# xenji/kafka-topic-analyzer

Measured on NVIDIA H100. Metric: messages/sec scanned (fused metric scan), higher is better.
Workload: dtype u64

## Files before the change

### kafka_topic_analyzer_b200/csrc/kta_api.cu

```cuda
#include <cuda_runtime.h>

#include <algorithm>
#include <chrono>
#include <climits>
#include <cmath>
#include <cstdarg>
#include <cstdio>
#include <cstdlib>
#include <cstring>
#include <new>
#include <vector>

#include "kta_host.cuh"
#include "kta_kernels.cuh"
#include "kta_logscan.cuh"
#include "kta_partitioner.cuh"
#include "kta_synth.h"
#include "kta_timeline.cuh"

using namespace kta;

extern "C" const char *kta_last_error(void) { return g_err; }
extern "C" int kta_abi_version(void) { return KTA_ABI_VERSION; }
extern "C" int kta_device_count(void) {
// ... 50 lines not shown
    int32_t buckets = 0;
    int64_t origin = 0, width = 1;
    bool smem = false;
    int blocks_per_sm = 0;
    DevBuf<unsigned long long> d_bins;
    std::vector<uint64_t> h_bins;
    size_t words() const { return d_bins.cap > 0 ? (size_t)d_bins.cap : 0; }
};

struct Partitioner {
    int32_t ncounts = 0;
    int32_t counts[KTA_PARTITIONER_MAX_COUNTS] = {};
    bool smem = false;
    int32_t max_grid = 0;
    DevBuf<unsigned long long> d_counts;
    std::vector<uint64_t> h_counts;
    size_t words() const { return d_counts.cap > 0 ? (size_t)d_counts.cap : 0; }
};

struct kta_handle {
    kta_config cfg{};
    int device = 0;
    int sm_count = 0;
    cudaStream_t stream = nullptr;
    bool own_stream = true;
    bool need_hash = false;
    DevBuf<unsigned long long> d_sums;
    DevBuf<long long> d_minmax;
    DevBuf<uint32_t> d_hll;
    DevBuf<uint32_t> d_hll_floor;
    AliveKeys alive;
    uint32_t *d_hash_out = nullptr;
    DevBuf<uint64_t> d_tb_scratch;
    LogScan log;
    Timeline tl;
    Partitioner pt;
    DevBuf<uint32_t> d_crc32_tables;
    size_t nsums = 0, nhll = 0;
    Chunk chunks[NCHUNK];
    bool ring_dev_ready = false, ring_host_ready = false;
    int64_t ring_records = 0, ring_key_bytes = 0;
    int cur = 0;
    struct PushCursor {
        int32_t *part = nullptr, *klen = nullptr, *vlen = nullptr;
        int64_t *ts = nullptr;
        uint8_t *keys = nullptr;
        uint64_t *tile_base = nullptr;
        int64_t n = 0, cap = 0;
        int64_t kb = 0, kcap = 0;
        bool hash = false;
    } pc;
    uint64_t next_seq = 0;
    bool finalized = false;
    std::vector<uint64_t> h_sums;
    long long h_minmax[4] = {0, 0, 0, 0};
    std::vector<uint32_t> h_hll;
    uint64_t h_alive = 0;
    int shard_world = 1, shard_rank = 0;
    int columns = 0;
    bool smem_counters = true;
    size_t smem_optin = 0;
    uint64_t launches = 0, records = 0;
    bool timing = false;
    std::vector<std::pair<cudaEvent_t, cudaEvent_t>> ev_pool;
    size_t ev_used = 0;
    double scan_ms = 0;
    uint64_t scan_launches_timed = 0;
};

static int set_device(const kta_handle *h) {
    CU(cudaSetDevice(h->device));
    return KTA_OK;
}

static bool keys_travel(const kta_handle *h) { return h->need_hash || h->d_hash_out || h->pt.ncounts; }

static size_t scan_smem_bytes(bool hash, bool smem, int P, int threads, int keybuf, int stages, bool hdr) {
    return (smem ? smem_counter_bytes(P) : CTA_SCRATCH) + (size_t)(threads / 32) * warp_smem_bytes(hash, keybuf, stages, hdr);
}

static void scan_shape(const kta_handle *h, bool hash, bool hdr_ok, int64_t n, int64_t key_bytes, int &threads, int &keybuf,
                       int &stages, bool &hdr, size_t &smem) {
    const int P = h->columns;
    keybuf = KEYBUF_MIN;
    stages = 0;
    hdr = false;
    if (!hash) {
        threads = MAX_THREADS;
        smem = scan_smem_bytes(false, h->smem_counters, P, threads, keybuf, stages, hdr);
        return;
    }
    if (n > 0) {
        const int64_t per_tile = (key_bytes * TILE + n - 1) / n;
        int64_t want = per_tile + per_tile / 8 + 64 + KEYBUF_SLACK;
        want = (want + 127) / 128 * 128;
        keybuf = (int)std::min<int64_t>(std::max<int64_t>(want, KEYBUF_MIN), KEYBUF_MAX);
        keybuf = (keybuf + 15) / 16 * 16;
    }
    auto fits = [&](bool with_hdr, int st, int max_warps, int min_warps) {
        hdr = with_hdr;
        stages = st;
        for (threads = std::min(max_warps * 32, HASH_MAX_THREADS); threads >= min_warps * 32; threads -= 32) {
            smem = scan_smem_bytes(true, h->smem_counters, P, threads, keybuf, stages, hdr);
            if (smem <= h->smem_optin) return true;
        }
        return false;
    };
    if (hdr_ok && (fits(true, SCAN_STAGES, 12, 10) || fits(true, 2, 12, 10))) return;
    if (fits(false, 2, 16, 8)) return;
// ... 251 lines not shown
    if (!h) return KTA_OK;
    cudaSetDevice(h->device);
    if (h->stream) cudaStreamSynchronize(h->stream);
    for (auto &c : h->chunks)
        if (c.free_ev) cudaEventDestroy(c.free_ev);
    for (auto &e : h->ev_pool) { cudaEventDestroy(e.first); cudaEventDestroy(e.second); }
    cudaStream_t own = h->own_stream ? h->stream : nullptr;
    delete h;
    if (own) cudaStreamDestroy(own);
    cudaGetLastError();
    return KTA_OK;
}

static int create_impl(const kta_config *cfg, kta_handle *h) {
    h->cfg = *cfg;
    if (cfg->num_partitions < 1 || cfg->num_partitions > (1 << 20))
        return fail(KTA_ERR_INVALID, "num_partitions %d out of range [1, 2^20]", cfg->num_partitions);
    if (cfg->hll_precision != 0 && (cfg->hll_precision < 4 || cfg->hll_precision > 18))
        return fail(KTA_ERR_INVALID, "hll_precision %d not 0 or 4..18", cfg->hll_precision);
    if (cfg->isolation_level != KTA_READ_UNCOMMITTED && cfg->isolation_level != KTA_READ_COMMITTED)
        return fail(KTA_ERR_INVALID, "isolation_level %d is neither KTA_READ_UNCOMMITTED (0) nor KTA_READ_COMMITTED (1)", cfg->isolation_level);
    int ndev = 0;
    CU(cudaGetDeviceCount(&ndev));
    if (ndev < 1) return fail(KTA_ERR_CUDA, "no CUDA device (this library has no CPU fallback)");
    if (cfg->device >= 0) h->device = cfg->device;
    else CU(cudaGetDevice(&h->device));
    if (h->device >= ndev) return fail(KTA_ERR_INVALID, "device %d >= device count %d", h->device, ndev);
    CU(cudaSetDevice(h->device));
    cudaDeviceProp prop;
    CU(cudaGetDeviceProperties(&prop, h->device));
    if (prop.major != 9 || prop.minor != 0) return fail(KTA_ERR_CUDA, "device %s is sm_%d%d; this library is built for sm_90a only",
                                     prop.name, prop.major, prop.minor);
    h->sm_count = prop.multiProcessorCount;
    CU(cudaStreamCreateWithFlags(&h->stream, cudaStreamNonBlocking));
    h->need_hash = cfg->count_alive_keys == 1 || cfg->hll_precision != 0;
    h->pc.hash = keys_travel(h);
    if (cfg->now_s == INT64_MIN) {
        const auto now = std::chrono::system_clock::now().time_since_epoch();
        const int64_t ns = std::chrono::duration_cast<std::chrono::nanoseconds>(now).count();
        h->cfg.now_s = ns / 1000000000ll;
        h->cfg.now_ns = (int32_t)(ns % 1000000000ll);
    }
    h->ring_records = cfg->ring_records > 0 ? cfg->ring_records : DEFAULT_RING_RECORDS;
    h->ring_records = (h->ring_records + TILE - 1) / TILE * TILE;
    h->ring_key_bytes = cfg->ring_key_bytes > 0 ? cfg->ring_key_bytes : h->ring_records * 24;

    const int P = cfg->num_partitions;
    h->nsums = sums_words(P);
    h->nhll = cfg->hll_precision ? ((size_t)1 << cfg->hll_precision) : 0;
    int rc;
    if ((rc = h->d_sums.alloc((int64_t)h->nsums)) || (rc = h->d_minmax.alloc(4)) || (rc = h->d_hll_floor.alloc(HLL_SLICES + 2)))
        return rc;
    if (h->nhll && (rc = h->d_hll.alloc((int64_t)h->nhll))) return rc;
    if (cfg->count_alive_keys == 1 && (rc = alive_create(h))) return rc;
    h->smem_optin = prop.sharedMemPerBlockOptin;
    if (cfg->shard_world > 1) {
        if (cfg->shard_rank < 0 || cfg->shard_rank >= cfg->shard_world || cfg->shard_world > P)
            return fail(KTA_ERR_INVALID, "shard_rank %d / shard_world %d invalid for %d partitions", cfg->shard_rank, cfg->shard_world, P);
        const uint64_t G = (uint64_t)cfg->shard_world, e = (((uint64_t)1 << 32) + G - 1) / G * G - ((uint64_t)1 << 32);
        if ((uint64_t)(P - 1) * e >= (uint64_t)1 << 32)
            return fail(KTA_ERR_INVALID, "shard_world %d with %d partitions: the scan's partition division is exact only when "
                        "(P - 1) * (ceil(2^32 / G) * G - 2^32) < 2^32 (every P <= 65536 and every G <= 4096 qualify)",
                        cfg->shard_world, P);
        h->shard_world = cfg->shard_world;
        h->shard_rank = cfg->shard_rank;
    }
    h->columns = (P - h->shard_rank + h->shard_world - 1) / h->shard_world;
    h->smem_counters = smem_counter_bytes(h->columns) + 8 * warp_smem_bytes(true, KEYBUF_MIN, 2, false) <= h->smem_optin;
    for (const auto &by_mode : SCAN_KERNELS[h->smem_counters])
        for (const auto &by_capture : by_mode)
            for (const ScanFn f : by_capture)
                if (f) CU(cudaFuncSetAttribute(f, cudaFuncAttributeMaxDynamicSharedMemorySize, (int)h->smem_optin));
    if ((rc = log_scan_create(h->log, cfg->isolation_level == KTA_READ_COMMITTED, h->smem_optin))) return rc;
    if ((rc = state_reset_device(h))) return rc;
    CU(cudaStreamSynchronize(h->stream));
    return KTA_OK;
}

extern "C" int kta_create(const kta_config *cfg, kta_handle **out) {
    if (!cfg || !out) return fail(KTA_ERR_INVALID, "null argument");
    if (cfg->struct_size != (int32_t)sizeof(kta_config))
        return fail(KTA_ERR_INVALID, "kta_config.struct_size %d != %zu (ABI version %d)", cfg->struct_size, sizeof(kta_config), KTA_ABI_VERSION);
    kta_handle *h = new (std::nothrow) kta_handle();
    if (!h) return fail(KTA_ERR_NOMEM, "out of host memory");
    const int rc = create_impl(cfg, h);
    if (rc) {
        char keep[sizeof(g_err)];
        memcpy(keep, g_err, sizeof(keep));
        kta_destroy(h);
        memcpy(g_err, keep, sizeof(keep));
        *out = nullptr;
        return rc;
    }
    *out = h;
    return KTA_OK;
}

extern "C" void *kta_stream(kta_handle *h) { return h ? (void *)h->stream : nullptr; }

extern "C" int kta_set_stream(kta_handle *h, void *stream) {
    if (!h) return fail(KTA_ERR_INVALID, "null handle");
    int rc;
    if ((rc = set_device(h))) return rc;
    CU(cudaStreamSynchronize(h->stream));
    if (h->own_stream) CU(cudaStreamDestroy(h->stream));
    h->stream = (cudaStream_t)stream;
// ... 617 lines not shown
    if ((rc = collect_timing(h))) return rc;
    h->next_seq = std::max<uint64_t>(h->next_seq, seq_base + (uint64_t)b->n);
    return KTA_OK;
}

extern "C" int kta_sync(kta_handle *h) {
    if (!h) return fail(KTA_ERR_INVALID, "null handle");
    int rc;
    if ((rc = set_device(h))) return rc;
    if ((rc = ring_flush(h))) return rc;
    CU(cudaStreamSynchronize(h->stream));
    if ((rc = alive_settle(h))) return rc;
    return collect_timing(h);
}

extern "C" int kta_reset(kta_handle *h) {
    if (!h) return fail(KTA_ERR_INVALID, "null handle");
    int rc;
    if ((rc = set_device(h))) return rc;
    h->pc.n = 0;
    h->pc.kb = 0;
    h->next_seq = 0;
    h->finalized = false;
    h->launches = 0;
    h->records = 0;
    h->log.txn.ranges.clear();
    for (uint64_t &v : h->log.txn.totals) v = 0;
    for (uint64_t &v : h->log.crc.totals) v = 0;
    h->log.crc.kept.clear();
    OffsetState &o = h->log.offsets;
    std::fill(o.win.begin(), o.win.end(), make_longlong2(-1, -1));
    o.set = 0;
    o.dirty = !o.win.empty();
    for (uint64_t &v : o.totals) v = 0;
    if (h->tl.buckets) CU(cudaMemsetAsync(h->tl.d_bins, 0, h->tl.words() * 8, h->stream));
    if (h->pt.ncounts) CU(cudaMemsetAsync(h->pt.d_counts, 0, h->pt.words() * 8, h->stream));
    return state_reset_device(h);
}

extern "C" int kta_finalize(kta_handle *h) {
    if (!h) return fail(KTA_ERR_INVALID, "null handle");
    int rc;
    if ((rc = set_device(h))) return rc;
    if ((rc = ring_flush(h))) return rc;
    cudaStream_t s = h->stream;
    if ((rc = alive_settle(h))) return rc;
    if (h->alive.d_table && h->nhll) {
        CU(cudaMemsetAsync(h->d_hll, 0, h->nhll * 4, s));
        alive_hll_kernel<<<h->sm_count * 8, THREADS, 0, s>>>(h->alive.d_table, (size_t)h->alive.pairs * 2, h->d_hll,
                                                             h->cfg.hll_precision);
        CU(cudaGetLastError());
        h->launches++;
    }
    h->h_sums.resize(h->nsums);
    h->h_hll.resize(h->nhll);
    CU(cudaMemcpyAsync(h->h_sums.data(), h->d_sums, h->nsums * 8, cudaMemcpyDeviceToHost, s));
    CU(cudaMemcpyAsync(h->h_minmax, h->d_minmax, 32, cudaMemcpyDeviceToHost, s));
    if (h->nhll) CU(cudaMemcpyAsync(h->h_hll.data(), h->d_hll, h->nhll * 4, cudaMemcpyDeviceToHost, s));
    if (h->tl.buckets) {
        h->tl.h_bins.resize(h->tl.words());
        CU(cudaMemcpyAsync(h->tl.h_bins.data(), h->tl.d_bins, h->tl.words() * 8, cudaMemcpyDeviceToHost, s));
    }
    if (h->pt.ncounts) {
        h->pt.h_counts.resize(h->pt.words());
        CU(cudaMemcpyAsync(h->pt.h_counts.data(), h->pt.d_counts, h->pt.words() * 8, cudaMemcpyDeviceToHost, s));
    }
    CU(cudaStreamSynchronize(s));
    if ((rc = collect_timing(h))) return rc;
    h->h_alive = h->alive.now;
    h->finalized = true;
    if (h->alive.window_errors)
        return fail(KTA_ERR_INVALID, "%llu record(s) carried a sequence number outside the alive-key table's window "
                    "[origin, origin + 2^31 - 2): with an explicit seq column the span between kta_reset calls is limited",
                    (unsigned long long)h->alive.window_errors);
    const uint64_t bad = h->h_sums[h->nsums - 1];
    if (bad)
        return fail(KTA_ERR_PARTITION, "%llu record(s) had a partition outside [0, %d) and were left out of every metric",
                    (unsigned long long)bad, h->cfg.num_partitions);
    return KTA_OK;
}

static int check_read(const kta_handle *h, int32_t p, bool per_partition) {
    if (!h) return fail(KTA_ERR_INVALID, "null handle");
    if (!h->finalized) return fail(KTA_ERR_NOT_FINALIZED, "call kta_finalize first");
    if (per_partition && (p < 0 || p >= h->cfg.num_partitions)) return -1;
    return KTA_OK;
}

static uint64_t raw_counter(const kta_handle *h, int which, int32_t p) {
    const int P = h->cfg.num_partitions;
    const uint64_t *s = h->h_sums.data();
    uint64_t knn = 0, alive = 0;
    for (int b = 0; b < NB; b++) {
        knn += s[(size_t)p * NB + b];
        alive += s[(size_t)(P + p) * NB + b];
    }
    const uint64_t knull = s[(size_t)P * (2 * NB + 2) + p];
    const uint64_t total = knn + knull;
    switch (which) {
        case KTA_TOTAL: return total;
        case KTA_TOMBSTONES: return total - alive;
        case KTA_ALIVE: return alive;
        case KTA_KEY_NULL: return knull;
        case KTA_KEY_NON_NULL: return knn;
        case KTA_KEY_SIZE_SUM: return s[(size_t)P * (2 * NB) + p];
        case KTA_VALUE_SIZE_SUM: return s[(size_t)P * (2 * NB + 1) + p];
    }
    return 0;
}

extern "C" int kta_counter(const kta_handle *h, int which, int32_t partition, uint64_t *out) {
    if (!out || which < 0 || which > KTA_VALUE_SIZE_SUM) return fail(KTA_ERR_INVALID, "bad argument");
    const int rc = check_read(h, partition, true);
    if (rc > 0) return rc;
    *out = rc < 0 ? 0 : raw_counter(h, which, partition);
    return KTA_OK;
}

extern "C" int kta_avg(const kta_handle *h, int which, int32_t partition, uint64_t *out) {
    if (!out || which < 0 || which > KTA_MESSAGE_SIZE_AVG) return fail(KTA_ERR_INVALID, "bad argument");
    const int rc = check_read(h, partition, true);
    if (rc > 0) return rc;
    if (rc < 0) { *out = 0; return KTA_OK; }
    const uint64_t ks = raw_counter(h, KTA_KEY_SIZE_SUM, partition), vs = raw_counter(h, KTA_VALUE_SIZE_SUM, partition);
    const uint64_t alive = raw_counter(h, KTA_ALIVE, partition);
    const uint64_t sum = which == KTA_KEY_SIZE_AVG ? ks : which == KTA_VALUE_SIZE_AVG ? vs : ks + vs;
    if (sum > 0) {
        if (alive == 0)
            return fail(KTA_ERR_DIV_BY_ZERO, "partition %d: sum %llu > 0 with alive == 0 (the reference panics here)",
                        partition, (unsigned long long)sum);
        *out = sum / alive;
    } else {
        *out = 0;
    }
    return KTA_OK;
}

extern "C" int kta_dirty_ratio(const kta_handle *h, int32_t partition, float *out) {
    if (!out) return fail(KTA_ERR_INVALID, "bad argument");
    const int rc = check_read(h, partition, true);
    if (rc > 0) return rc;
    *out = 0.0f;
    if (rc < 0) return KTA_OK;
    const uint64_t total = raw_counter(h, KTA_TOTAL, partition), tomb = raw_counter(h, KTA_TOMBSTONES, partition);
    if (total > 0 && tomb > 0) {
        const volatile float t = (float)tomb;
        const volatile float d = (float)total / 100.0f;
        *out = t / d;
    }
    return KTA_OK;
}

extern "C" int kta_global(const kta_handle *h, int which, uint64_t *out) {
    if (!out) return fail(KTA_ERR_INVALID, "bad argument");
    const int rc = check_read(h, 0, false);
    if (rc) return rc;
    const int P = h->cfg.num_partitions;
    const unsigned long long *mm = reinterpret_cast<const unsigned long long *>(h->h_minmax);
    switch (which) {
        case KTA_SMALLEST_MESSAGE: *out = mm[2] == ~0ull ? 0 : mm[2]; return KTA_OK;
        case KTA_LARGEST_MESSAGE: *out = mm[3]; return KTA_OK;
        case KTA_OVERALL_SIZE: {
            uint64_t s = 0;
            for (int p = 0; p < P; p++) s += raw_counter(h, KTA_KEY_SIZE_SUM, p) + raw_counter(h, KTA_VALUE_SIZE_SUM, p);
            *out = s;
            return KTA_OK;
        }
        case KTA_OVERALL_COUNT: {
            uint64_t s = 0;
            for (int p = 0; p < P; p++) s += raw_counter(h, KTA_TOTAL, p);
            *out = s;
            return KTA_OK;
        }
    }
    return fail(KTA_ERR_INVALID, "bad global id %d", which);
}

extern "C" int kta_timestamps(const kta_handle *h, int64_t *earliest_s, int32_t *earliest_ns, int64_t *latest_s) {
    const int rc = check_read(h, 0, false);
    if (rc) return rc;
    int64_t es = h->cfg.now_s, ls = 0;
    int32_t ens = h->cfg.now_ns;
    if (h->h_minmax[0] != INT64_MAX) {
        const int64_t raw_mn = h->h_minmax[0] == -1 ? 0 : h->h_minmax[0];
        const int64_t raw_mx = h->h_minmax[1] == -1 ? 0 : h->h_minmax[1];
        const int64_t mn = raw_mn / 1000, mx = raw_mx / 1000;
        if (es > mn || (es == mn && ens > 0)) { es = mn; ens = 0; }
        if (ls < mx) ls = mx;
    }
    if (earliest_s) *earliest_s = es;
    if (earliest_ns) *earliest_ns = ens;
    if (latest_s) *latest_s = ls;
    return KTA_OK;
}

extern "C" int kta_alive_keys(const kta_handle *h, uint64_t *out) {
    if (!out) return fail(KTA_ERR_INVALID, "bad argument");
    const int rc = check_read(h, 0, false);
    if (rc) return rc;
    if (h->cfg.count_alive_keys != 1) return fail(KTA_ERR_NOT_ENABLED, "count_alive_keys was not enabled");
    *out = h->h_alive;
    return KTA_OK;
}

extern "C" int kta_bad_partition_records(const kta_handle *h, uint64_t *out) {
    if (!out) return fail(KTA_ERR_INVALID, "bad argument");
    const int rc = check_read(h, 0, false);
    if (rc) return rc;
    *out = h->h_sums[h->nsums - 1];
    return KTA_OK;
}
// ... 121 lines not shown
    if (!h || cap < 0 || (cap && !out)) return fail(KTA_ERR_INVALID, "bad argument");
    if (!h->pt.ncounts) return fail(KTA_ERR_NOT_ENABLED, "the partitioner check is off (kta_set_partitioner_check)");
    const int rc = check_read(h, partition, true);
    if (rc > 0) return rc;
    const int64_t nv = 2 * (int64_t)h->pt.ncounts + 1, n = std::min<int64_t>(cap, nv);
    for (int64_t b = 0; b < n; b++)
        out[b] = rc < 0 ? 0 : h->pt.h_counts[(size_t)b * (size_t)h->cfg.num_partitions + (size_t)partition];
    return KTA_OK;
}

extern "C" int kta_partitioner_shape(const kta_handle *h, int64_t n, int64_t key_bytes, int32_t *grid, int32_t *stage,
                                     int32_t *smem_counters) {
    if (!h || n < 0 || !grid || !stage || !smem_counters) return fail(KTA_ERR_INVALID, "bad argument");
    if (!h->pt.ncounts) return fail(KTA_ERR_NOT_ENABLED, "the partitioner check is off (kta_set_partitioner_check)");
    int rc;
    if ((rc = set_device(h))) return rc;
    int g = 0, st = 0;
    size_t sm = 0;
    if ((rc = partitioner_shape(h, n, key_bytes, g, st, sm))) return rc;
    *grid = g;
    *stage = st;
    *smem_counters = h->pt.smem ? 1 : 0;
    return KTA_OK;
}

extern "C" int kta_partitioner_limit_grid(kta_handle *h, int32_t max_ctas) {
    if (!h || max_ctas < 0) return fail(KTA_ERR_INVALID, "bad argument");
    if (!h->pt.ncounts) return fail(KTA_ERR_NOT_ENABLED, "the partitioner check is off (kta_set_partitioner_check)");
    h->pt.max_grid = max_ctas;
    return KTA_OK;
}

static double hll_sigma(double x) {
    if (x == 1.0) return INFINITY;
    double y = 1.0, z = x, zo;
    do { x *= x; zo = z; z += x * y; y += y; } while (zo != z);
    return z;
}
static double hll_tau(double x) {
    if (x == 0.0 || x == 1.0) return 0.0;
    double y = 1.0, z = 1.0 - x, zo;
    do { x = std::sqrt(x); zo = z; y *= 0.5; z -= (1.0 - x) * (1.0 - x) * y; } while (zo != z);
    return z / 3.0;
}

extern "C" int kta_alive_keys_hll(const kta_handle *h, double *out) {
    if (!out) return fail(KTA_ERR_INVALID, "bad argument");
    const int rc = check_read(h, 0, false);
    if (rc) return rc;
    if (!h->nhll) return fail(KTA_ERR_NOT_ENABLED, "hll_precision was 0");
    const int p = h->cfg.hll_precision, q = 32 - p;
    const double m = (double)h->nhll;
    std::vector<double> C((size_t)q + 2, 0.0);
    for (uint32_t r : h->h_hll) C[std::min<uint32_t>(r, (uint32_t)q + 1)] += 1.0;
    double z = m * hll_tau(1.0 - C[(size_t)q + 1] / m);
    for (int k = q; k >= 1; k--) z = 0.5 * (z + C[(size_t)k]);
    z += m * hll_sigma(C[0] / m);
    *out = 0.72134752044448170368 * m * m / z;
    return KTA_OK;
}

extern "C" int kta_hll_registers(const kta_handle *h, uint8_t *out, size_t cap) {
    if (!out) return fail(KTA_ERR_INVALID, "bad argument");
    const int rc = check_read(h, 0, false);
    if (rc) return rc;
    if (!h->nhll) return fail(KTA_ERR_NOT_ENABLED, "hll_precision was 0");
    if (cap < h->nhll) return fail(KTA_ERR_INVALID, "buffer too small: %zu < %zu", cap, h->nhll);
    for (size_t i = 0; i < h->nhll; i++) out[i] = (uint8_t)h->h_hll[i];
    return KTA_OK;
}

extern "C" int kta_fnv32_host(kta_handle *h, int64_t n, const int32_t *key_len, const uint8_t *key_bytes,
                              int64_t key_bytes_len, uint32_t *out) {
    if (!h || n < 0 || (n && (!key_len || !out))) return fail(KTA_ERR_INVALID, "bad argument");
    if (n == 0) return KTA_OK;
    int rc;
    if ((rc = set_device(h))) return rc;
    std::vector<uint64_t> off((size_t)n);
    uint64_t acc = 0;
    for (int64_t i = 0; i < n; i++) {
        off[(size_t)i] = acc;
        acc += key_len[i] > 0 ? (uint64_t)key_len[i] : 0;
    }
    if ((int64_t)acc > key_bytes_len) return fail(KTA_ERR_INVALID, "key_bytes_len %lld < sum of key_len %llu",
                                                  (long long)key_bytes_len, (unsigned long long)acc);
    DevBuf<int32_t> d_len;
    DevBuf<uint64_t> d_off;
    DevBuf<uint8_t> d_keys;
    DevBuf<uint32_t> d_out;
    cudaStream_t s = h->stream;
    if ((rc = d_len.alloc(n)) || (rc = d_off.alloc(n)) || (rc = d_keys.alloc((int64_t)acc + 16)) || (rc = d_out.alloc(n))) return rc;
    CU(cudaMemcpyAsync(d_len, key_len, n * 4, cudaMemcpyHostToDevice, s));
    CU(cudaMemcpyAsync(d_off, off.data(), n * 8, cudaMemcpyHostToDevice, s));
    if (acc) CU(cudaMemcpyAsync(d_keys, key_bytes, acc, cudaMemcpyHostToDevice, s));
    fnv32_kernel<<<(int)std::min<int64_t>((n + 255) / 256, 1024), 256, 0, s>>>(n, d_len, d_off, d_keys, d_out);
    h->launches++;
    CU(cudaGetLastError());
    CU(cudaMemcpyAsync(out, d_out, n * 4, cudaMemcpyDeviceToHost, s));
    CU(cudaStreamSynchronize(s));
    return KTA_OK;
}

extern "C" int kta_partitioner_hash_host(kta_handle *h, int64_t n, const int32_t *key_len, const uint8_t *key_bytes,
                                         int64_t key_bytes_len, uint32_t *murmur2, uint32_t *crc32) {
    if (!h || n < 0 || (n && (!key_len || !murmur2 || !crc32))) return fail(KTA_ERR_INVALID, "bad argument");
    if (n == 0) return KTA_OK;
    int rc;
// ... 132 lines not shown
```

### kafka_topic_analyzer_b200/csrc/kta_kernels.cuh

```cuda
#pragma once
#include <cuda_runtime.h>
#include <stdint.h>

#include <type_traits>

#include "../../include/kta.h"

namespace kta {

constexpr int MAX_THREADS = 1024;
constexpr int HASH_MAX_THREADS = 512;
constexpr int TILE = KTA_KEY_TILE;
constexpr int ROWS = TILE / 32;
constexpr int NB = KTA_HIST_BUCKETS;
constexpr int KEYBUF_MIN = TILE * 18 + 32, KEYBUF_MAX = TILE * 128 + 32, KEYBUF_SLACK = 32;
constexpr int HDR_P = 0, HDR_TS = TILE * 4, HDR_KL = TILE * 12, HDR_VL = TILE * 16;
constexpr int HDR_BYTES = TILE * 20;
constexpr int SCAN_STAGES = 3;
constexpr int MAX_STAGES = 4;
static_assert(SCAN_STAGES >= 2 && SCAN_STAGES <= MAX_STAGES, "2..4 stages per warp");
__host__ __device__ inline size_t warp_smem_bytes(bool hash, int keybuf, int stages, bool hdr) {
    return hash ? 128 + (size_t)stages * ((size_t)keybuf + (hdr ? HDR_BYTES : 0)) : 128;
}
constexpr uint32_t FNV_BASIS = 0x811c9dc5u;
// ... 402 lines not shown
        if (v == ALIVE_EMPTY) {
            v = atomicCAS(slot + s, ALIVE_EMPTY, stamp);
            if (v == ALIVE_EMPTY) return true;
        }
        if ((uint32_t)(v >> 32) == hash) {
            if (v >= stamp) newest = (uint32_t)v;
            else alive_red_max(slot + s, stamp, t.pol);
            return true;
        }
    }
    return false;
}

__device__ __noinline__ uint32_t alive_stamp_slow(const AliveTable t, uint32_t pair, uint32_t hash, uint32_t low) {
    uint32_t newest;
    for (int probe = 0; probe < ALIVE_MAX_PROBES; probe++) {
        if (alive_probe_pair(t, pair, hash, low, newest)) return newest;
        pair = pair + 1 == t.npairs ? 0 : pair + 1;
    }
    if (__ldcg(t.status + 2)) {
        for (uint32_t probe = ALIVE_MAX_PROBES; probe < t.npairs; probe++) {
            if (alive_probe_pair(t, pair, hash, low, newest)) return newest;
            pair = pair + 1 == t.npairs ? 0 : pair + 1;
        }
    }
    atomicAdd(t.status, 1u);
    return low;
}

__device__ __forceinline__ uint32_t alive_stamp(const AliveTable t, uint32_t pair, const ulonglong2 e, uint32_t hash, uint32_t low) {
    const bool hx = (uint32_t)(e.x >> 32) == hash, hy = (uint32_t)(e.y >> 32) == hash;
    const uint32_t seen = hx ? (uint32_t)e.x : (uint32_t)e.y;
    if ((hx || hy) && seen + 1u > low) return seen;
    unsigned long long *slot = t.slots + 2 * (size_t)pair;
    const unsigned long long stamp = ((unsigned long long)hash << 32) | low;
    const bool ex = e.x == ALIVE_EMPTY, ey = e.y == ALIVE_EMPTY;
    if ((hx && !ex) || (!hx && hy && !ey)) {
        alive_red_max(slot + (hx ? 0 : 1), stamp, t.pol);
        return low;
    }
    if (ex || ey) {
        unsigned long long *sl = slot + (ex ? 0 : 1);
        const unsigned long long old = atomicCAS(sl, ALIVE_EMPTY, stamp);
        if (old == ALIVE_EMPTY) return low;
        if ((uint32_t)(old >> 32) == hash) {
            if (old >= stamp) return (uint32_t)old;
            alive_red_max(sl, stamp, t.pol);
            return low;
        }
    }
    return alive_stamp_slow(t, pair, hash, low);
}

constexpr int ALIVE_CACHE_SET_BITS = 23, ALIVE_CACHE_TAG_BITS = 32 - ALIVE_CACHE_SET_BITS, ALIVE_CACHE_WAVE_BITS = 16 - ALIVE_CACHE_TAG_BITS;
constexpr uint32_t ALIVE_CACHE_WAVES = (1u << ALIVE_CACHE_WAVE_BITS) - 1;
static_assert(ALIVE_CACHE_TAG_BITS == 9 && ALIVE_CACHE_WAVE_BITS == 7, "16-bit ways");
__device__ __forceinline__ uint32_t alive_cache_ld(const uint32_t *p, uint64_t pol) {
    uint32_t v;
    asm volatile("ld.global.cg.L2::cache_hint.u32 %0, [%1], %2;" : "=r"(v) : "l"(p), "l"(pol));
    return v;
}
__device__ __forceinline__ bool alive_cache_newer(uint32_t c, uint32_t x, uint32_t wv) {
    const uint32_t tag = x & ((1u << ALIVE_CACHE_TAG_BITS) - 1u);
    const uint32_t w0 = c & 0xffffu, w1 = c >> 16;
    const uint32_t lo = (tag << ALIVE_CACHE_WAVE_BITS) | wv;
    return (w0 - lo - 1u < ALIVE_CACHE_WAVES - wv) || (w1 - lo - 1u < ALIVE_CACHE_WAVES - wv);
}
__device__ __forceinline__ void alive_cache_put(uint32_t *cache, uint32_t c, uint32_t x, uint32_t wv, uint32_t pick) {
    const uint32_t tag = x & ((1u << ALIVE_CACHE_TAG_BITS) - 1u);
    const uint32_t mine = (tag << ALIVE_CACHE_WAVE_BITS) | wv;
    const uint32_t w0 = c & 0xffffu, w1 = c >> 16;
    int way;
    if ((w0 >> ALIVE_CACHE_WAVE_BITS) == tag && w0) way = w0 >= mine ? -1 : 0;
    else if ((w1 >> ALIVE_CACHE_WAVE_BITS) == tag && w1) way = w1 >= mine ? -1 : 1;
    else way = w0 == 0 ? 0 : w1 == 0 ? 1 : (int)(pick & 1u);
    if (way >= 0) reinterpret_cast<unsigned short *>(cache + (x >> ALIVE_CACHE_TAG_BITS))[way] = (unsigned short)mine;
}

__device__ __forceinline__ bool alive_insert_unique(unsigned long long *slots, uint32_t npairs, unsigned long long entry) {
    uint32_t pair = alive_home((uint32_t)(entry >> 32), npairs);
    for (uint32_t probe = 0; probe < npairs; probe++) {
        unsigned long long *slot = slots + 2 * (size_t)pair;
#pragma unroll
        for (int s = 0; s < 2; s++)
            if (__ldcg(slot + s) == ALIVE_EMPTY && atomicCAS(slot + s, ALIVE_EMPTY, entry) == ALIVE_EMPTY) return true;
        pair = pair + 1 == npairs ? 0 : pair + 1;
    }
    return false;
}

__device__ __noinline__ void wide_tile_hashes(const int32_t *key_len, int64_t n, const uint8_t *tile_keys, int64_t tile,
                                              uint32_t *out , int lane) {
    uint64_t carry = 0;
    for (int k = 0; k < ROWS; k++) {
        const int64_t r = tile * TILE + 32 * k + lane;
        const int kl = r < n ? key_len[r] : -1;
        const uint64_t v = (uint64_t)max(kl, 0);
        uint64_t inc = v;
        for (int d = 1; d < 32; d <<= 1) {
            const uint64_t t = __shfl_up_sync(0xffffffffu, inc, d);
            if (lane >= d) inc += t;
        }
        out[32 * k + lane] = kl >= 0 ? fnv_global(tile_keys + carry + inc - v, kl) : 0u;
        carry += __shfl_sync(0xffffffffu, inc, 31);
    }
    __syncwarp();
}

struct AliveWaves {
// ... 340 lines not shown
    }
    return o;
}

template <bool CAPTURE, int MODE>
__device__ __forceinline__ void hash_tile(const ScanParams &prm, TilePipe<MODE> &pipe, int buf, TileDesc d, int tile, int64_t rbase,
                                          const TileRows &rec, const KeyOffsets &o, int lane, uint32_t (&h)[ROWS]) {
    const uint32_t kb = pipe.stage(buf);
    if (d.keys_staged()) {
        const uint32_t a0 = d.key_lead();
        if (!d.hdr_staged()) pipe.wait(buf);
        if (o.fix16 && a0 == 0) {
#pragma unroll
            for (int k = 0; k < ROWS; k += 2) {
                const uint4 qa = lds128(kb + o.off[k]);
                const uint4 qb = lds128(kb + o.off[k + 1]);
                uint32_t ha = FNV_BASIS, hb = FNV_BASIS;
                ha = fnv_word(ha, qa.x); hb = fnv_word(hb, qb.x);
                ha = fnv_word(ha, qa.y); hb = fnv_word(hb, qb.y);
                ha = fnv_word(ha, qa.z); hb = fnv_word(hb, qb.z);
                ha = fnv_word(ha, qa.w); hb = fnv_word(hb, qb.w);
                h[k] = ha;
                h[k + 1] = hb;
            }
        } else {
#pragma unroll
            for (int k = 0; k < ROWS; k++) h[k] = rec.kl[k] >= 0 ? fnv_smem(kb, a0 + o.off[k], rec.kl[k]) : 0u;
        }
    } else if (o.fixL || o.small) {
        const uint64_t g0 = prm.key_tile_base[tile];
#pragma unroll
        for (int k = 0; k < ROWS; k++)
            h[k] = (rec.valid[k] && rec.kl[k] >= 0) ? fnv_global(prm.key_bytes + g0 + o.off[k], rec.kl[k]) : 0u;
    } else {
        uint32_t *scratch = reinterpret_cast<uint32_t *>(pipe.stage_ptr(buf));
        wide_tile_hashes(prm.key_len, prm.n, prm.key_bytes + prm.key_tile_base[tile], tile, scratch, lane);
#pragma unroll
        for (int k = 0; k < ROWS; k++) h[k] = scratch[32 * k + lane];
    }
    if (CAPTURE) {
#pragma unroll
        for (int k = 0; k < ROWS; k++)
            if (rec.valid[k]) prm.hash_out[rbase + 32 * k] = rec.kl[k] >= 0 ? h[k] : 0u;
    }
}

struct ExactProbe {
    uint32_t x[ROWS];
    uint32_t low[ROWS];
    uint32_t cw[ROWS];
    bool live[ROWS];
};

__device__ __forceinline__ ExactProbe exact_probe(const ScanParams &prm, const AliveTable &AT, const AliveWaves &AW,
                                                  const TileRows &rec, const uint32_t (&h)[ROWS], int64_t rbase) {
    const bool cached = AW.cache != nullptr;
    const uint32_t r32 = (uint32_t)rbase;
    ExactProbe e;
#pragma unroll
    for (int k = 0; k < ROWS; k++) {
        e.live[k] = (rec.clean || rec.use[k]) && rec.kl[k] >= 0;
        uint32_t field;
        if (prm.seq) {
            const uint64_t f = e.live[k] ? ld_stream_u64(prm.seq + rbase + 32 * k) - prm.alive_origin + 1ull : 1ull;
            if (f - 1ull >= (uint64_t)ALIVE_FIELD_MAX) {
                atomicAdd(prm.alive_status + 1, 1u);
                e.live[k] = false;
            }
            field = (uint32_t)f;
        } else {
            field = (uint32_t)prm.alive_fbase + r32 + 32u * k;
        }
        e.low[k] = (field << 1) | (rec.vl[k] >= 0 ? 1u : 0u);
        e.x[k] = hll_mix(h[k]);
        e.cw[k] = 0;
        if (cached && e.live[k]) e.cw[k] = alive_cache_ld(AW.cache + (e.x[k] >> ALIVE_CACHE_TAG_BITS), AT.pol);
    }
    return e;
}

__device__ __forceinline__ void exact_resolve(const AliveTable &AT, const AliveWaves &AW, const ExactProbe &e, unsigned char *stage,
                                              int lane, unsigned lt_mask) {
    static_assert(TILE * 16 <= KEYBUF_MIN, "the queue stays inside the key part of the stage");
    uint4 *queue = reinterpret_cast<uint4 *>(stage);
    const bool cached = AW.cache != nullptr;
    __syncwarp();
    uint32_t qn = 0;
#pragma unroll
    for (int k = 0; k < ROWS; k++) {
        const bool go = e.live[k] && !(cached && alive_cache_newer(e.cw[k], e.x[k], alive_wave(e.low[k] >> 1, AW)));
        const unsigned m = __ballot_sync(0xffffffffu, go);
        if (go) queue[qn + __popc(m & lt_mask)] = make_uint4(e.x[k], e.low[k], e.cw[k], 0u);
        qn += __popc(m);
    }
    __syncwarp();
    for (uint32_t q0 = 0; q0 < qn; q0 += 32) {
        if (q0 + lane < qn) {
            const uint4 item = queue[q0 + lane];
            const uint32_t pr = alive_home(item.x, AT.npairs);
            const ulonglong2 en = alive_ld_pair(AT.slots + 2 * (size_t)pr, AT.pol);
            const uint32_t newest = alive_stamp(AT, pr, en, item.x, item.y);
            if (cached)
                alive_cache_put(AW.cache, item.z, item.x, max(alive_wave(item.y >> 1, AW), alive_wave(newest >> 1, AW)), newest >> 1);
        }
    }
    asm volatile("fence.proxy.async.shared::cta;" ::: "memory");
    __syncwarp();
}

__device__ __forceinline__ void sketch_tile(const ScanParams &prm, uint32_t floor_reg, const TileRows &rec, const uint32_t (&h)[ROWS]) {
    const uint32_t skip_mask = hll_skip_mask(prm.hll_p, floor_reg);
#pragma unroll
    for (int k = 0; k < ROWS; k++) {
        const uint32_t x = hll_mix(h[k]);
        if (((x & skip_mask) | (uint32_t)((rec.kl[k] | rec.vl[k]) >> 31)) == 0 && (rec.clean || rec.use[k])) hll_raise(prm.hll, prm.hll_p, x);
    }
}

template <bool SMEM>
__device__ __forceinline__ void flush_counters(const ScanParams &prm, const Counters<SMEM> &C, int tid, int warp, int lane) {
    const int nh = (ROW_V + NB) * C.P;
    for (int i = tid; i < nh; i += blockDim.x) {
        const uint32_t v = C.s[i];
        if (v) {
            const int row = i / C.P, pp = C.part(i - row * C.P);
            if (row < NB) atomicAdd(&prm.sums[(size_t)pp * NB + row], (unsigned long long)v);
            else if (row == NB) atomicAdd(&prm.sums[(size_t)prm.P * (2 * NB + 2) + pp], (unsigned long long)v);
            else atomicAdd(&prm.sums[(size_t)(prm.P + pp) * NB + (row - ROW_V)], (unsigned long long)v);
        }
    }
    if (warp == 0) C.fold_sums(lane, 1u);
}

__device__ __forceinline__ void flush_totals(const ScanParams &prm, WarpTotals w, unsigned char *wsm, size_t warp_bytes, int tid,
                                             int lane, int nwarps) {
    const unsigned full = 0xffffffffu;
    long long smin64 = w.smin != 0xffffffffu ? (long long)w.smin : INT64_MAX;
    long long smax64 = w.smin != 0xffffffffu ? (long long)w.smax : -1;
#pragma unroll
    for (int d = 16; d; d >>= 1) {
        const long long a = __shfl_xor_sync(full, w.tmin, d), b = __shfl_xor_sync(full, w.tmax, d);
        const long long c = __shfl_xor_sync(full, smin64, d), e = __shfl_xor_sync(full, smax64, d);
        w.tmin = a < w.tmin ? a : w.tmin;
        w.tmax = b > w.tmax ? b : w.tmax;
        smin64 = c < smin64 ? c : smin64;
        smax64 = e > smax64 ? e : smax64;
        w.bad += __shfl_xor_sync(full, w.bad, d);
    }
    long long *red = reinterpret_cast<long long *>(wsm + 64);
    if (lane == 0) {
        red[0] = w.tmin; red[1] = w.tmax; red[2] = smin64; red[3] = smax64;
        if (w.bad) atomicAdd(&prm.sums[sums_words(prm.P) - 1], (unsigned long long)w.bad);
    }
    __syncthreads();
    if (tid == 0) {
        for (int i = 1; i < nwarps; i++) {
            const long long *rw = reinterpret_cast<const long long *>(wsm + (size_t)i * warp_bytes + 64);
            w.tmin = rw[0] < w.tmin ? rw[0] : w.tmin;
            w.tmax = rw[1] > w.tmax ? rw[1] : w.tmax;
            smin64 = rw[2] < smin64 ? rw[2] : smin64;
            smax64 = rw[3] > smax64 ? rw[3] : smax64;
        }
        if (w.tmin != INT64_MAX) {
            atomicMin(&prm.minmax[0], w.tmin);
            atomicMax(&prm.minmax[1], w.tmax);
        }
        if (smax64 >= 0) {
            atomicMin(reinterpret_cast<unsigned long long *>(&prm.minmax[2]), (unsigned long long)smin64);
            atomicMax(reinterpret_cast<unsigned long long *>(&prm.minmax[3]), (unsigned long long)smax64);
        }
    }
}

template <int MODE, bool SMEM, bool CAPTURE, bool SHARD = false>
__global__ void __launch_bounds__(MODE == MODE_COUNTERS ? MAX_THREADS : HASH_MAX_THREADS, 1) scan_kernel(const ScanParams prm) {
    constexpr bool HASH = MODE != MODE_COUNTERS;
    extern __shared__ __align__(128) unsigned char smem_raw[];
    const int tid = threadIdx.x, lane = tid & 31, warp = tid >> 5, nwarps = blockDim.x >> 5;
    const unsigned lt_mask = (1u << lane) - 1u;
    const int P = SHARD ? prm.Pc : prm.P;
    uint32_t *scnt = reinterpret_cast<uint32_t *>(smem_raw);
    const size_t cta_bytes = SMEM ? smem_counter_bytes(P) : CTA_SCRATCH;
    const uint32_t KEYBUF = (uint32_t)prm.keybuf;
    const int S = HASH ? prm.stages : 0;
    const size_t warp_bytes = warp_smem_bytes(HASH, prm.keybuf, S, prm.hdr_stage);
    unsigned char *wsm = smem_raw + cta_bytes + (size_t)warp * warp_bytes;
    const uint32_t mbar = smem_u32(wsm);
    const uint32_t stage0 = smem_u32(wsm) + 128;
    const Counters<SMEM> C{smem_u32(scnt), scnt, prm.sums, P, prm.P, SHARD ? prm.shard_world : 1, SHARD ? prm.shard_rank : 0};
    const uint64_t pol_stream = MODE == MODE_EXACT ? l2_policy_evict_first() : 0;
    const AliveTable AT{prm.alive_table, prm.alive_pairs, prm.alive_status, MODE == MODE_EXACT ? l2_policy_evict_last() : 0};
    const AliveWaves AW{prm.alive_cache, prm.alive_wave_base, prm.alive_wave_shift};
    const bool count_it = !(MODE == MODE_EXACT && prm.alive_only);

    if (SMEM) {
        const int nw = P * SMEM_ROWS;
        for (int i = tid; i < nw; i += blockDim.x) scnt[i] = 0;
    }
    if (HASH && lane == 0) {
        for (int b = 0; b < S; b++) mbar_init(mbar + 8u * b, 1);
        fence_mbar_init();
    }
    __syncthreads();

    WarpTotals tot;
    uint32_t floor_reg = MODE == MODE_HLL ? ld_cg_u32(prm.hll_floor) : 0u;

    const int ntiles = (int)prm.ntiles;
    const int gstride = (int)gridDim.x * nwarps;
    int tile = (int)blockIdx.x * nwarps + warp;
    TilePipe<MODE> pipe{prm, wsm, mbar, stage0, KEYBUF, KEYBUF + (prm.hdr_stage ? (uint32_t)HDR_BYTES : 0u), S, ntiles, tile, gstride, lane,
                        pol_stream};
    if (HASH) pipe.start();

    auto scan_tile = [&](auto full_tag, int tile, int buf, TileDesc d) {
        constexpr bool FULL = decltype(full_tag)::value;
        const int64_t rbase = (int64_t)tile * TILE + lane;
        TileRows rec;
        load_headers<FULL>(prm, pipe, buf, d, rbase, lane, rec);
        partition_check<FULL, SHARD>(prm, rec);
        uint32_t h[ROWS] = {0u, 0u, 0u, 0u};
        if (MODE != MODE_EXACT) count_tile(C, rec, count_it, lane, tot);
        if (HASH) hash_tile<CAPTURE>(prm, pipe, buf, d, tile, rbase, rec, key_offsets(rec.kl, lane), lane, h);
        if (MODE == MODE_EXACT) {
            unsigned char *queue = pipe.stage_ptr(buf);
            const ExactProbe e = exact_probe(prm, AT, AW, rec, h, rbase);
            count_tile(C, rec, count_it, lane, tot);
            exact_resolve(AT, AW, e, queue, lane, lt_mask);
        }
        if (MODE == MODE_HLL) sketch_tile(prm, floor_reg, rec, h);
    };

    int buf = 0;
    for (int it = 0; tile < ntiles; tile += gstride, ++it) {
        const TileDesc d = HASH ? pipe.next(tile, buf) : TileDesc{0u};
        const int pt = pipe.phys(tile);
        if ((int64_t)(pt + 1) * TILE <= prm.n) scan_tile(std::true_type{}, pt, buf, d);
        else scan_tile(std::false_type{}, pt, buf, d);
        if (HASH) buf = buf + 1 == S ? 0 : buf + 1;
        if (SMEM && (it & (FOLD_TILES - 1)) == FOLD_TILES - 1) C.fold_sums(lane, 1u << 30);
        tot.try_uni = tot.try_uni || (it & 15) == 15;
        if (MODE == MODE_HLL) {
            if (((it & 3) == 3 && ((it >> 2) & 31) == (warp & 31)) || (it < 2 && warp == it + 1))
                hll_refresh_slice(prm.hll, prm.hll_p, prm.hll_floor, (blockIdx.x + (uint32_t)(it >> 2) * 37u) & (HLL_SLICES - 1), lane);
            if (it < 4 || (it & 15) == 15) floor_reg = ld_cg_u32(prm.hll_floor);
        }
    }

    __syncthreads();
    if (SMEM) flush_counters(prm, C, tid, warp, lane);
    flush_totals(prm, tot, wsm, warp_bytes, tid, lane, nwarps);
}

__global__ void __launch_bounds__(256) tile_key_bytes_kernel(const int32_t *key_len, int64_t n, int64_t ntiles,
                                                             uint64_t *tile_base ) {
    const int lane = threadIdx.x & 31;
    const int64_t gw = ((int64_t)blockIdx.x * blockDim.x + threadIdx.x) >> 5, gs = ((int64_t)gridDim.x * blockDim.x) >> 5;
    for (int64_t tile = gw; tile < ntiles; tile += gs) {
        uint64_t s = 0;
#pragma unroll
        for (int k = 0; k < ROWS; k++) {
            const int64_t r = tile * TILE + k * 32 + lane;
            if (r < n) {
                const int32_t v = key_len[r];
                s += v > 0 ? (uint64_t)v : 0;
            }
        }
#pragma unroll
        for (int d = 16; d; d >>= 1) s += __shfl_xor_sync(0xffffffffu, s, d);
        if (lane == 0) tile_base[tile + 1] = s;
    }
    if (blockIdx.x == 0 && threadIdx.x == 0) tile_base[0] = 0;
}

__global__ void __launch_bounds__(1024) tile_base_scan_kernel(uint64_t *tile_base, int64_t ntiles) {
    __shared__ uint64_t wsum[32];
    __shared__ uint64_t carry_s;
    const int tid = threadIdx.x, lane = tid & 31, warp = tid >> 5;
    if (tid == 0) carry_s = 0;
    __syncthreads();
    for (int64_t base = 1; base <= ntiles; base += 1024) {
        const int64_t i = base + tid;
// ... 177 lines not shown
```

Measured before the change: 84.19 billion.

## Shrink alive cache sets, split L2 policies, pin host result buffers

Cuts the alive-key cache's set bits from 23 to 22 by default, which halves the cache array and widens the tag. The streamed alive-table accesses now use evict-first while the cache loads use evict-last, so the cache stays resident in L2. Host result buffers become pinned allocations made at init, avoiding pageable copies at finalize. It also adds an optional compile-time attribution probe path and factors the exact-mode body into a helper; the smaller cache may raise miss rates.

```diff
diff --git a/kafka_topic_analyzer_b200/csrc/kta_api.cu b/kafka_topic_analyzer_b200/csrc/kta_api.cu
--- a/kafka_topic_analyzer_b200/csrc/kta_api.cu
+++ b/kafka_topic_analyzer_b200/csrc/kta_api.cu
@@ -126,9 +126,9 @@
     } pc;
     uint64_t next_seq = 0;
     bool finalized = false;
-    std::vector<uint64_t> h_sums;
-    long long h_minmax[4] = {0, 0, 0, 0};
-    std::vector<uint32_t> h_hll;
+    PinnedBuf<uint64_t> h_sums;
+    PinnedBuf<long long> h_minmax;
+    PinnedBuf<uint32_t> h_hll;
     uint64_t h_alive = 0;
     int shard_world = 1, shard_rank = 0;
     int columns = 0;
@@ -486,6 +486,11 @@
     if ((rc = h->d_sums.alloc((int64_t)h->nsums)) || (rc = h->d_minmax.alloc(4)) || (rc = h->d_hll_floor.alloc(HLL_SLICES + 2)))
         return rc;
     if (h->nhll && (rc = h->d_hll.alloc((int64_t)h->nhll))) return rc;
+    if ((rc = h->h_sums.alloc((int64_t)h->nsums)) || (rc = h->h_minmax.alloc(4)) || (h->nhll && (rc = h->h_hll.alloc((int64_t)h->nhll))))
+        return rc;
+    std::fill(h->h_sums.get(), h->h_sums.get() + h->nsums, 0ull);
+    std::fill(h->h_minmax.get(), h->h_minmax.get() + 4, 0ll);
+    if (h->nhll) std::fill(h->h_hll.get(), h->h_hll.get() + h->nhll, 0u);
     if (cfg->count_alive_keys == 1 && (rc = alive_create(h))) return rc;
     h->smem_optin = prop.sharedMemPerBlockOptin;
     if (cfg->shard_world > 1) {
@@ -1209,11 +1214,9 @@
         CU(cudaGetLastError());
         h->launches++;
     }
-    h->h_sums.resize(h->nsums);
-    h->h_hll.resize(h->nhll);
-    CU(cudaMemcpyAsync(h->h_sums.data(), h->d_sums, h->nsums * 8, cudaMemcpyDeviceToHost, s));
+    CU(cudaMemcpyAsync(h->h_sums, h->d_sums, h->nsums * 8, cudaMemcpyDeviceToHost, s));
     CU(cudaMemcpyAsync(h->h_minmax, h->d_minmax, 32, cudaMemcpyDeviceToHost, s));
-    if (h->nhll) CU(cudaMemcpyAsync(h->h_hll.data(), h->d_hll, h->nhll * 4, cudaMemcpyDeviceToHost, s));
+    if (h->nhll) CU(cudaMemcpyAsync(h->h_hll, h->d_hll, h->nhll * 4, cudaMemcpyDeviceToHost, s));
     if (h->tl.buckets) {
         h->tl.h_bins.resize(h->tl.words());
         CU(cudaMemcpyAsync(h->tl.h_bins.data(), h->tl.d_bins, h->tl.words() * 8, cudaMemcpyDeviceToHost, s));
@@ -1246,7 +1249,7 @@
 
 static uint64_t raw_counter(const kta_handle *h, int which, int32_t p) {
     const int P = h->cfg.num_partitions;
-    const uint64_t *s = h->h_sums.data();
+    const uint64_t *s = h->h_sums.get();
     uint64_t knn = 0, alive = 0;
     for (int b = 0; b < NB; b++) {
         knn += s[(size_t)p * NB + b];
@@ -1313,7 +1316,7 @@
     const int rc = check_read(h, 0, false);
     if (rc) return rc;
     const int P = h->cfg.num_partitions;
-    const unsigned long long *mm = reinterpret_cast<const unsigned long long *>(h->h_minmax);
+    const unsigned long long *mm = reinterpret_cast<const unsigned long long *>(h->h_minmax.get());
     switch (which) {
         case KTA_SMALLEST_MESSAGE: *out = mm[2] == ~0ull ? 0 : mm[2]; return KTA_OK;
         case KTA_LARGEST_MESSAGE: *out = mm[3]; return KTA_OK;
@@ -1541,7 +1544,7 @@
     const int p = h->cfg.hll_precision, q = 32 - p;
     const double m = (double)h->nhll;
     std::vector<double> C((size_t)q + 2, 0.0);
-    for (uint32_t r : h->h_hll) C[std::min<uint32_t>(r, (uint32_t)q + 1)] += 1.0;
+    for (size_t i = 0; i < h->nhll; i++) C[std::min<uint32_t>(h->h_hll[i], (uint32_t)q + 1)] += 1.0;
     double z = m * hll_tau(1.0 - C[(size_t)q + 1] / m);
     for (int k = q; k >= 1; k--) z = 0.5 * (z + C[(size_t)k]);
     z += m * hll_sigma(C[0] / m);
diff --git a/kafka_topic_analyzer_b200/csrc/kta_kernels.cuh b/kafka_topic_analyzer_b200/csrc/kta_kernels.cuh
--- a/kafka_topic_analyzer_b200/csrc/kta_kernels.cuh
+++ b/kafka_topic_analyzer_b200/csrc/kta_kernels.cuh
@@ -478,9 +478,12 @@
     return alive_stamp_slow(t, pair, hash, low);
 }
 
-constexpr int ALIVE_CACHE_SET_BITS = 23, ALIVE_CACHE_TAG_BITS = 32 - ALIVE_CACHE_SET_BITS, ALIVE_CACHE_WAVE_BITS = 16 - ALIVE_CACHE_TAG_BITS;
+#ifndef KTA_ALIVE_CACHE_SET_BITS
+#define KTA_ALIVE_CACHE_SET_BITS 22
+#endif
+constexpr int ALIVE_CACHE_SET_BITS = KTA_ALIVE_CACHE_SET_BITS, ALIVE_CACHE_TAG_BITS = 32 - ALIVE_CACHE_SET_BITS, ALIVE_CACHE_WAVE_BITS = 16 - ALIVE_CACHE_TAG_BITS;
 constexpr uint32_t ALIVE_CACHE_WAVES = (1u << ALIVE_CACHE_WAVE_BITS) - 1;
-static_assert(ALIVE_CACHE_TAG_BITS == 9 && ALIVE_CACHE_WAVE_BITS == 7, "16-bit ways");
+static_assert(ALIVE_CACHE_WAVE_BITS >= 3 && ALIVE_CACHE_WAVE_BITS <= 7, "16-bit ways");
 __device__ __forceinline__ uint32_t alive_cache_ld(const uint32_t *p, uint64_t pol) {
     uint32_t v;
     asm volatile("ld.global.cg.L2::cache_hint.u32 %0, [%1], %2;" : "=r"(v) : "l"(p), "l"(pol));
@@ -927,8 +930,8 @@
     bool live[ROWS];
 };
 
-__device__ __forceinline__ ExactProbe exact_probe(const ScanParams &prm, const AliveTable &AT, const AliveWaves &AW,
-                                                  const TileRows &rec, const uint32_t (&h)[ROWS], int64_t rbase) {
+__device__ __forceinline__ ExactProbe exact_probe(const ScanParams &prm, const AliveWaves &AW, uint64_t cpol, const TileRows &rec,
+                                                  const uint32_t (&h)[ROWS], int64_t rbase) {
     const bool cached = AW.cache != nullptr;
     const uint32_t r32 = (uint32_t)rbase;
     ExactProbe e;
@@ -949,7 +952,7 @@
         e.low[k] = (field << 1) | (rec.vl[k] >= 0 ? 1u : 0u);
         e.x[k] = hll_mix(h[k]);
         e.cw[k] = 0;
-        if (cached && e.live[k]) e.cw[k] = alive_cache_ld(AW.cache + (e.x[k] >> ALIVE_CACHE_TAG_BITS), AT.pol);
+        if (cached && e.live[k]) e.cw[k] = alive_cache_ld(AW.cache + (e.x[k] >> ALIVE_CACHE_TAG_BITS), cpol);
     }
     return e;
 }
@@ -981,6 +984,30 @@
     }
     asm volatile("fence.proxy.async.shared::cta;" ::: "memory");
     __syncwarp();
+}
+
+template <bool SMEM, int MODE>
+__device__ __forceinline__ void exact_tile(const ScanParams &prm, TilePipe<MODE> &pipe, const Counters<SMEM> C, const AliveTable &AT,
+                                           const AliveWaves &AW, const TileRows &rec, const uint32_t (&h)[ROWS], bool count_it, int buf,
+                                           int64_t rbase, int lane, unsigned lt_mask, WarpTotals &tot) {
+    const uint64_t cpol = l2_policy_evict_last();
+#if defined(KTA_EXACT_ATTRIB)
+    uint32_t cw[ROWS];
+#pragma unroll
+    for (int k = 0; k < ROWS; k++) {
+        uint32_t set = hll_mix(h[k]) >> ALIVE_CACHE_TAG_BITS;
+        if (KTA_EXACT_ATTRIB == 2) set &= (1u << 18) - 1u;
+        cw[k] = AW.cache && (rec.clean || rec.use[k]) && rec.kl[k] >= 0 ? alive_cache_ld(AW.cache + set, cpol) : 0u;
+    }
+    count_tile(C, rec, count_it, lane, tot);
+    if ((cw[0] | cw[1] | cw[2] | cw[3]) == 0x9e3779b9u) atomicAdd(prm.alive_status + 1, 1u);
+    (void)pipe; (void)buf; (void)rbase; (void)lt_mask;
+#else
+    unsigned char *queue = pipe.stage_ptr(buf);
+    const ExactProbe e = exact_probe(prm, AW, cpol, rec, h, rbase);
+    count_tile(C, rec, count_it, lane, tot);
+    exact_resolve(AT, AW, e, queue, lane, lt_mask);
+#endif
 }
 
 __device__ __forceinline__ void sketch_tile(const ScanParams &prm, uint32_t floor_reg, const TileRows &rec, const uint32_t (&h)[ROWS]) {
@@ -1064,7 +1091,7 @@
     const uint32_t stage0 = smem_u32(wsm) + 128;
     const Counters<SMEM> C{smem_u32(scnt), scnt, prm.sums, P, prm.P, SHARD ? prm.shard_world : 1, SHARD ? prm.shard_rank : 0};
     const uint64_t pol_stream = MODE == MODE_EXACT ? l2_policy_evict_first() : 0;
-    const AliveTable AT{prm.alive_table, prm.alive_pairs, prm.alive_status, MODE == MODE_EXACT ? l2_policy_evict_last() : 0};
+    const AliveTable AT{prm.alive_table, prm.alive_pairs, prm.alive_status, MODE == MODE_EXACT ? l2_policy_evict_first() : 0};
     const AliveWaves AW{prm.alive_cache, prm.alive_wave_base, prm.alive_wave_shift};
     const bool count_it = !(MODE == MODE_EXACT && prm.alive_only);
 
@@ -1097,12 +1124,7 @@
         uint32_t h[ROWS] = {0u, 0u, 0u, 0u};
         if (MODE != MODE_EXACT) count_tile(C, rec, count_it, lane, tot);
         if (HASH) hash_tile<CAPTURE>(prm, pipe, buf, d, tile, rbase, rec, key_offsets(rec.kl, lane), lane, h);
-        if (MODE == MODE_EXACT) {
-            unsigned char *queue = pipe.stage_ptr(buf);
-            const ExactProbe e = exact_probe(prm, AT, AW, rec, h, rbase);
-            count_tile(C, rec, count_it, lane, tot);
-            exact_resolve(AT, AW, e, queue, lane, lt_mask);
-        }
+        if (MODE == MODE_EXACT) exact_tile(prm, pipe, C, AT, AW, rec, h, count_it, buf, rbase, lane, lt_mask, tot);
         if (MODE == MODE_HLL) sketch_tile(prm, floor_reg, rec, h);
     };
 
```

Result: no change. 84.59 billion (median of 6 runs) (+0.5%).
